# muhanzhang/IGMC

Measured on AMD Instinct MI355X. Metric: enclosing-subgraphs/sec (train step, batch=50) + test RMSE, higher is better.
Workload: dtype f32; 1 GPU; ml_1m, hop 1, max-nodes-per-hop 100, batch 50 per GPU, adj-dropout 0, dynamic-train, ARR 0.001, Adam; parallelism=dp1, global_batch=50, graphs_captured_before_timing=True, steps_per_graph_launch=100, group_steps=50

## Files before the change

### igmc_amd/csrc/capi.hip

```cpp
#include "launch.h"
#include "sortpool.h"
#include "g2_image.h"

#include <algorithm>
#include <climits>
#include <cmath>
#include <cstdio>
#include <cstring>
#include <map>
#include <string>
#include <vector>

static thread_local std::string g_err;
int g_igmc_prof_on = 0;

#define IGMC_FAIL(msg)                                                      \
  do {                                                                      \
    g_err = std::string(__func__) + ": " + (msg);                           \
    return 1;                                                               \
  } while (0)
#define HIPCHECK(expr)                                                      \
  do {                                                                      \
    hipError_t e_ = (expr);                                                 \
    if (e_ != hipSuccess) {                                                 \
// ... 467 lines not shown
      IGMC_FAIL("group extraction needs lean arenas with one control block attached and no side-feature source");
  }
  igmc_launch_extract_set(g->d, s->d_views, b0->d, count, d_link_u, d_link_v, d_link_y, d_link_idx, sel0, B, sample_ratio,
                          seed, b0->ctrl, drop_p, force_undirected, drop_seed, stream);
  HIPCHECK(hipGetLastError());
  for (int i = 0; i < count; ++i) s->arenas[i]->last_B = B;
  return 0;
}

static void ensure_csr(const igmc_batch* b, void* stream) {
  if (b->lean && b->d.relm && b->last_B > 0) igmc_launch_emit(b->d, b->last_B, stream);
}

extern "C" int igmc_batch_assume_size(igmc_batch* b, int B) {
  if (!b) IGMC_FAIL("null batch");
  if (B <= 0 || B > b->d.graph_cap) IGMC_FAIL("batch size out of range");
  b->last_B = B;
  return 0;
}

extern "C" int igmc_batch_set_lean(igmc_batch* b, int lean) {
  if (!b) IGMC_FAIL("null batch");
  b->lean = lean ? 1 : 0;
  return 0;
}

extern "C" int igmc_batch_edge_dropout(igmc_batch* b, float p, int force_undirected, uint64_t seed, uint64_t step,
                                       void* stream) {
  if (!b) IGMC_FAIL("null batch");
  if (b->lean && b->d.relm && b->last_B > 0) {
    igmc_launch_relm_dropout(b->d, b->last_B, p, force_undirected, seed, step, b->ctrl, stream);
  } else {
    igmc_launch_edge_flags(b->d, p, force_undirected, seed, step, b->ctrl, stream);
  }
  HIPCHECK(hipGetLastError());
  return 0;
}

extern "C" int igmc_batch_get_info(const igmc_batch* b, igmc_batch_info* out, void* stream) {
  if (!b || !out) IGMC_FAIL("null argument");
  ensure_csr(b, stream);
  int32_t t[8];
  HIPCHECK(hipStreamSynchronize((hipStream_t)stream));
  HIPCHECK(hipMemcpy(t, b->d.totals, sizeof(t), hipMemcpyDeviceToHost));
  out->num_graphs = t[3];
  out->num_nodes = t[2] ? t[4] : t[0];
  out->num_edges = t[2] ? t[5] : t[1];
  out->overflow = t[2];
  out->node_capacity = b->d.node_cap;
  out->edge_capacity = b->d.edge_cap;
  out->num_labels = b->d.num_labels;
  out->hop = b->d.hop;
  return 0;
}

extern "C" int igmc_batch_set_edge_flags(igmc_batch* b, const uint8_t* h_flags, int64_t n) {
  if (!b || !h_flags) IGMC_FAIL("null argument");
  if (n > b->d.edge_cap) IGMC_FAIL("too many flags");
  ensure_csr(b, nullptr);
  HIPCHECK(hipDeviceSynchronize());
  HIPCHECK(hipMemcpy(b->d.eflag, h_flags, (size_t)n, hipMemcpyHostToDevice));
  igmc_launch_relm_flags(b->d, nullptr);
  HIPCHECK(hipDeviceSynchronize());
  return 0;
}

extern "C" int igmc_batch_clear_edge_flags(igmc_batch* b) {
  if (!b) IGMC_FAIL("null batch");
  igmc_batch_info info;
  if (igmc_batch_get_info(b, &info, nullptr)) return 1;
  if (info.num_edges > 0) {
    HIPCHECK(hipMemset(b->d.eflag, 3, (size_t)info.num_edges));
    igmc_launch_relm_flags(b->d, nullptr);
    HIPCHECK(hipDeviceSynchronize());
  }
  return 0;
}

extern "C" int igmc_batch_download(const igmc_batch* b, int32_t* node_off, int32_t* n_users, uint8_t* node_label,
                                   int32_t* node_gid, int32_t* node_graph, int32_t* row_ptr, int32_t* col,
                                   uint8_t* erel, uint8_t* elab, uint8_t* eflag, float* y, void* stream) {
  igmc_batch_info info;
  if (igmc_batch_get_info(b, &info, stream)) return 1;
  if (info.overflow) IGMC_FAIL("batch arena overflow");
  const int B = info.num_graphs, N = info.num_nodes, E = info.num_edges;
  const BatchDev& d = b->d;
  if (node_off) HIPCHECK(hipMemcpy(node_off, d.node_off, (B + 1) * 4, hipMemcpyDeviceToHost));
  if (n_users) HIPCHECK(hipMemcpy(n_users, d.n_users, B * 4, hipMemcpyDeviceToHost));
  if (node_label && N) HIPCHECK(hipMemcpy(node_label, d.node_label, N, hipMemcpyDeviceToHost));
  if (node_gid && N) HIPCHECK(hipMemcpy(node_gid, d.node_gid, N * 4, hipMemcpyDeviceToHost));
  if (node_graph && N) HIPCHECK(hipMemcpy(node_graph, d.node_graph, N * 4, hipMemcpyDeviceToHost));
  if (row_ptr) HIPCHECK(hipMemcpy(row_ptr, d.row_ptr, (N + 1) * 4, hipMemcpyDeviceToHost));
  if ((col || erel) && E) {
    std::vector<uint32_t> ecr(E);
    HIPCHECK(hipMemcpy(ecr.data(), d.ecr, (size_t)E * 4, hipMemcpyDeviceToHost));
    for (int e = 0; e < E; ++e) {
      if (col) col[e] = (int32_t)(ecr[e] & 0xFFFFFFu);
      if (erel) erel[e] = (uint8_t)(ecr[e] >> 24);
    }
  }
  if (elab && E) {
    std::vector<uint16_t> code(E);
    HIPCHECK(hipMemcpy(code.data(), d.ecode, (size_t)E * 2, hipMemcpyDeviceToHost));
    for (int e = 0; e < E; ++e) elab[e] = (uint8_t)(code[e] % d.num_labels);
  }
  if (eflag && E) HIPCHECK(hipMemcpy(eflag, d.eflag, E, hipMemcpyDeviceToHost));
  if (y) HIPCHECK(hipMemcpy(y, d.y, B * sizeof(float), hipMemcpyDeviceToHost));
  return 0;
}

extern "C" void* igmc_batch_device_ptr(const igmc_batch* b, int which) {
  if (!b) return nullptr;
  const BatchDev& d = b->d;
  switch (which) {
    case IGMC_BUF_NODE_OFF: return d.node_off;
    case IGMC_BUF_N_USERS: return d.n_users;
    case IGMC_BUF_NODE_LABEL: return d.node_label;
    case IGMC_BUF_NODE_GID: return d.node_gid;
    case IGMC_BUF_NODE_GRAPH: return d.node_graph;
    case IGMC_BUF_ROW_PTR: return d.row_ptr;
    case IGMC_BUF_ECR: return d.ecr;
    case IGMC_BUF_ECODE: return d.ecode;
    case IGMC_BUF_EFLAG: return d.eflag;
    case IGMC_BUF_Y: return d.y;
    case IGMC_BUF_TOTALS: return d.totals;
  }
  return nullptr;
}

extern "C" int igmc_batch_set_side_features(igmc_batch* b, const float* d_feat, int n_side) {
  if (!b) IGMC_FAIL("null batch");
  b->side = d_feat;
  b->n_side = n_side;
  b->side_src = nullptr;
  return 0;
}

extern "C" int igmc_batch_bind_side_source(igmc_batch* b, const float* d_side_all, int n_side) {
  if (!b) IGMC_FAIL("null batch");
  if (!d_side_all || n_side <= 0) {
    b->side_src = nullptr;
    b->side = nullptr;
    b->n_side = 0;
    return 0;
  }
  if (b->side_buf_cols < n_side) {
    HIPCHECK(hipSetDevice(b->g->device));
    const int cols = std::max(n_side, 2 * b->side_buf_cols);
    if (b->mem.get(&b->side_buf, (size_t)b->d.graph_cap * cols)) IGMC_FAIL("hipMalloc failed (side features)");
    b->side_buf_cols = cols;
  }
  b->side_src = d_side_all;
  b->side = b->side_buf;
  b->n_side = n_side;
  return 0;
}

extern "C" int igmc_model_create(int device, int num_relations, int num_bases, int num_labels, int n_side,
                                 int max_nodes, int max_edges, int max_graphs, igmc_model** out) {
  if (!out) IGMC_FAIL("null out");
  if (num_bases != 4) IGMC_FAIL("the gfx950 kernels are built for num_bases == 4 (reference Main.py:393)");
  if (num_relations < 1 || num_relations > 255) IGMC_FAIL("num_relations out of range");
  if (num_relations * num_labels + num_labels + 1 > 320) IGMC_FAIL("num_relations * num_labels too large for the layer-0 gradient kernel");
  if (num_labels < 2 || n_side < 0 || max_nodes < 1 || max_graphs < 1) IGMC_FAIL("bad sizes");
  HIPCHECK(hipSetDevice(device));
  igmc_model* m = new igmc_model();
  m->device = device;
  m->last_B = 0;
  m->last_training = 0;
  m->last_flags = 0;
  m->img_valid = 0;
  m->img_hint = 0;
  m->img_params = nullptr;
  ModelDev& d = m->d;
  d.img_current = 0;
  d.adam_m1 = nullptr;
  d.adam_m2 = nullptr;
  d.R = num_relations;
  d.Bs = 4;
  d.L = num_labels;
  d.S = n_side;
  d.D = 256 + n_side;
  int64_t off = 0;
  for (int l = 0; l < 4; ++l) {
    const int fin = l == 0 ? d.L : 32;
    d.off_basis[l] = off; off += (int64_t)4 * fin * 32;
    d.off_root[l] = off;  off += (int64_t)fin * 32;
    d.off_bias[l] = off;  off += 32;
    d.off_att[l] = off;   off += (int64_t)d.R * 4;
  }
  d.off_l1w = off; off += (int64_t)128 * d.D;
  d.off_l1b = off; off += 128;
  d.off_l2w = off; off += 128;
  d.off_l2b = off; off += 1;
  d.n_params = off;
  d.node_cap = max_nodes;
  d.edge_cap = max_edges;
  d.graph_cap = max_graphs;
  Allocs& M = m->mem;
  int fail = 0;
  const size_t N = (size_t)max_nodes, Bc = (size_t)max_graphs;
  for (int l = 0; l < 4; ++l) fail |= M.get(&d.h[l], N * 32) | M.get(&d.dpre[l], N * 32);
  fail |= M.get(&d.agg, N * 128);
  for (int l = 0; l < 3; ++l) fail |= M.get(&d.gagg[l], N * 128) | M.get(&d.Y[l], N * 128);
  fail |= M.get(&d.feat, Bc * d.D) | M.get(&d.a1, Bc * 128) | M.get(&d.lmask, Bc * 128) | M.get(&d.dz, Bc * 128) |
          M.get(&d.gfeat, Bc * d.D) | M.get(&d.err, Bc) | M.get(&d.cnt0, N * d.R * d.L);
  const size_t rows0 = (size_t)d.R * d.L + d.L + 1;
  d.ts_part = nullptr;
  d.ts_raw = nullptr;
  d.ts_stride = (d.R * 32 + 33) * 32;
  d.fin_stash = nullptr;
  d.datt_part = nullptr;
  if (d.R <= G2_NR * G2_NG_MAX)
  {
    fail |= M.get(&d.ts_part, (size_t)4 * IGMC_TS_BLOCKS * d.ts_stride) |
            M.get(&d.ts_raw, (size_t)4 * d.ts_stride + (size_t)4 * d.ts_stride / 32 * 4);
    if (!fail) d.datt_part = d.ts_raw + (size_t)4 * d.ts_stride;
  }
  if (d.R <= 128) fail |= M.get(&d.fin_stash, (size_t)4 * IGMC_STASH_LAYER + 16);
  d.g2_ex = nullptr;
  d.g2_fx = nullptr;
  d.g2_px = nullptr;
  d.g2_px_stride = 0;
  d.g2_w = nullptr;
  d.g2_graphs = 0;
  d.ex_nodes = 256;
  d.g2_ex_stride = (size_t)Bc * 2 * 32 * d.ex_nodes;
  const int wide = d.R <= G2_NR * G2_NG_MAX;
  const int xcd_ok = igmc_g2_xcd_ok();
  if (wide && Bc <= 2048 && xcd_ok) {
    fail |= M.get(&d.g2_ex, 5 * d.g2_ex_stride) | M.get(&d.g2_fx, Bc * 256) | M.get(&d.g2_w, g2_w_words(d.R, d.L));
    d.g2_graphs = (int)Bc;
    if (d.R <= G2_NR && Bc <= 1024) {
      d.g2_px_stride = (size_t)Bc * 2 * 32768;
      fail |= M.get(&d.g2_px, 5 * d.g2_px_stride);
    } else if (d.R <= G2_NR) {
      static bool told = false;
      if (!told) fprintf(stderr, "[igmc] batches of more than 1024 subgraphs: no plane-exchange regions -- the dense-layer / per-layer kernels take the steps, not the subgraph kernel\n");
      told = true;
    }
  } else if (wide) {
    fail |= M.get(&d.g2_w, g2_w_words(d.R, d.L));
  }
  fail |= M.get(&d.gs_bar, 2 * Bc + 1);
  fail |= M.get(&d.gs_ts, 4);
  d.gs_err = d.gs_bar ? d.gs_bar + 2 * Bc : nullptr;
  fail |= M.get(&d.wg_part, (size_t)4 * IGMC_WG_BLOCKS * igmc_wg_stride()) |
          M.get(&d.gatt_part, (size_t)3 * IGMC_GATHER_BLOCKS * d.R * 4) |
          M.get(&d.l0_part, (size_t)IGMC_L0_BLOCKS * rows0 * 32) |
          M.get(&d.graw, (size_t)3 * igmc_wg_stride() + 3 * d.R * 4 + rows0 * 32) | M.get(&d.arr_part, 4);
  d.side = nullptr;
  d.ctrl = nullptr;
  d.dcat[0] = d.dcat[1] = d.dcat[2] = nullptr;
  fail |= M.get(&m->done_ctr, 8);
  if (fail) {
    M.release();
    delete m;
    IGMC_FAIL("hipMalloc failed (model workspace)");
  }
  {
    hipStream_t st1, st2;
    if (hipStreamCreateWithFlags(&st1, hipStreamNonBlocking) != hipSuccess ||
        hipStreamCreateWithFlags(&st2, hipStreamNonBlocking) != hipSuccess) {
      M.release();
      delete m;
      IGMC_FAIL("hipStreamCreate failed");
    }
    m->ax.s1 = st1;
    m->ax.s2 = st2;
    for (int i = 0; i < 8; ++i) {
      hipEvent_t e;
      if (hipEventCreateWithFlags(&e, hipEventDisableTiming) != hipSuccess) IGMC_FAIL("hipEventCreate failed");
      m->ax.ev[i] = e;
    }
  }
  HIPCHECK(hipMemset(m->done_ctr, 0, 8 * sizeof(int)));
  HIPCHECK(hipMemset(m->d.gs_bar, 0, (2 * (size_t)max_graphs + 1) * sizeof(int)));
  {
    const unsigned long long ts0[4] = {~0ull, 0ull, 0ull, 0ull};
    HIPCHECK(hipMemcpy(m->d.gs_ts, ts0, sizeof(ts0), hipMemcpyHostToDevice));
  }
  if (m->d.g2_ex) {
    HIPCHECK(hipMemset(m->d.g2_ex, 0, 5 * m->d.g2_ex_stride * sizeof(unsigned long long)));
    HIPCHECK(hipMemset(m->d.g2_fx, 0, (size_t)max_graphs * 256 * sizeof(unsigned long long)));
    if (m->d.g2_px) HIPCHECK(hipMemset(m->d.g2_px, 0, 5 * m->d.g2_px_stride));
  }
  if (igmc_model_prepare(d)) {
    M.release();
    delete m;
    IGMC_FAIL("hipFuncSetAttribute failed");
  }
  *out = m;
  return 0;
}

extern "C" int igmc_debug_lin_mask(const igmc_model* m, uint8_t* h_out, int64_t n) {
  if (!m || !h_out) IGMC_FAIL("null argument");
  if (n < 0 || n > (int64_t)m->d.graph_cap * 128) IGMC_FAIL("mask size out of range");
  HIPCHECK(hipDeviceSynchronize());
  HIPCHECK(hipMemcpy(h_out, m->d.lmask, (size_t)n, hipMemcpyDeviceToHost));
  return 0;
}

extern "C" void igmc_model_destroy(igmc_model* m) {
  if (!m) return;
  for (int i = 0; i < 8; ++i) hipEventDestroy((hipEvent_t)m->ax.ev[i]);
  hipStreamDestroy((hipStream_t)m->ax.s1);
  hipStreamDestroy((hipStream_t)m->ax.s2);
  m->mem.release();
  delete m;
}

extern "C" int64_t igmc_param_count(const igmc_model* m) { return m ? m->d.n_params : 0; }

extern "C" int64_t igmc_param_offset(const igmc_model* m, int layer, int which, int64_t* count) {
  if (!m) return -1;
  const ModelDev& d = m->d;
  const int fin = (layer == 0) ? d.L : 32;
  int64_t off = -1, n = 0;
  switch (which) {
    case IGMC_P_BASIS: off = d.off_basis[layer & 3]; n = (int64_t)4 * fin * 32; break;
    case IGMC_P_ROOT: off = d.off_root[layer & 3]; n = (int64_t)fin * 32; break;
    case IGMC_P_BIAS: off = d.off_bias[layer & 3]; n = 32; break;
    case IGMC_P_ATT: off = d.off_att[layer & 3]; n = (int64_t)d.R * 4; break;
    case IGMC_P_LIN1_W: off = d.off_l1w; n = (int64_t)128 * d.D; break;
    case IGMC_P_LIN1_B: off = d.off_l1b; n = 128; break;
    case IGMC_P_LIN2_W: off = d.off_l2w; n = 128; break;
    case IGMC_P_LIN2_B: off = d.off_l2b; n = 1; break;
  }
  if (count) *count = n;
  return off;
}

static StepPlan plan_query(const igmc_model* m, const igmc_batch* b, int B) {
  StepPlan sp;
  igmc_step_plan(m->d, b->d, B, IGMC_CALL_STEP, &sp);
  return sp;
}

extern "C" int igmc_model_dense_layers(const igmc_model* m, const igmc_batch* b, int B) {
  return (m && b) ? plan_query(m, b, B).dense_layers : 0;
}

extern "C" int igmc_model_dense_path(const igmc_model* m, const igmc_batch* b, int B) {
  return (m && b) ? plan_query(m, b, B).family == IGMC_FAM_G2 : 0;
}

extern "C" int igmc_model_step_form(const igmc_model* m, const igmc_batch* b, int B) {
  return (m && b) ? plan_query(m, b, B).step_form : 0;
}

extern "C" int igmc_model_step_geometry(const igmc_model* m, const igmc_batch* b, int B, int32_t* out, int n) {
  if (!m || !b || !out || n < 0) IGMC_FAIL("bad arguments");
  if (B < 1 || B > b->d.graph_cap) IGMC_FAIL("batch size outside the arena's capacity");
  const StepPlan sp = plan_query(m, b, B);
  const int g2 = sp.family == IGMC_FAM_G2, dense = sp.family == IGMC_FAM_DLF || sp.family == IGMC_FAM_DL;
  const int32_t v[IGMC_GEOM_N] = {sp.step_form,
                                  sp.family,
                                  g2 ? sp.cs : 0,
                                  g2 ? sp.grid : 0,
                                  sp.nqu,
                                  sp.nqv,
                                  sp.family == IGMC_FAM_ROWS ? 0 : sp.wide ? g2_groups(m->d.R, m->d.L) : 1,
                                  sp.wide && sp.gsplit,
                                  g2 || sp.dlts,
                                  g2 ? sp.lay.kp : 0,
                                  dense && sp.dlb};
  for (int i = 0; i < n && i < IGMC_GEOM_N; ++i) out[i] = v[i];
  return 0;
}

static int check_fit(igmc_model* m, const igmc_batch* b, std::string* why) {
  if (!m || !b) { *why = "null model or batch"; return 1; }
  if (b->last_B <= 0) { *why = "batch is empty (run igmc_extract_batch first)"; return 1; }
  if (b->d.node_cap > m->d.node_cap || b->d.graph_cap > m->d.graph_cap) { *why = "batch capacity exceeds the model workspace"; return 1; }
  if (b->d.num_labels != m->d.L) { *why = "num_labels mismatch (hop)"; return 1; }
  if (b->g->max_rel >= m->d.R) { *why = "graph has more relations than the model"; return 1; }
  if (m->d.S != b->n_side && m->d.S > 0) { *why = "side feature width mismatch"; return 1; }
  return 0;
}

static int check_call(igmc_model* m, const igmc_batch* b, bool buffers, std::string* why) {
  if (check_fit(m, b, why)) return 1;
  if (!buffers) { *why = "null buffer"; return 1; }
  return 0;
}
static StepPlan begin_call(igmc_model* m, const igmc_batch* b, int kind, void* stream) {
  m->d.side = b->side;
  StepPlan sp;
  igmc_step_plan(m->d, b->d, b->last_B, kind, &sp);
  if (b->lean && sp.needs_csr) ensure_csr(b, stream);
  return sp;
}
static void end_call(igmc_model* m, const igmc_batch* b, int training, int use_edge_flags) {
  m->last_B = b->last_B;
  m->last_training = training;
  m->last_flags = use_edge_flags;
}

struct AdamScalars {
  float step_size, inv_sqrt_bc2;
};
static AdamScalars adam_scalars(const int64_t* d_ctrl, int64_t t, float lr, float beta1, float beta2) {
  AdamScalars a = {0.f, 0.f};
  if (!d_ctrl) {
    const double bc1 = 1.0 - std::pow((double)beta1, (double)t);
    const double bc2 = 1.0 - std::pow((double)beta2, (double)t);
    a.step_size = (float)((double)lr / bc1);
    a.inv_sqrt_bc2 = (float)(1.0 / std::sqrt(bc2));
  }
  return a;
}

extern "C" int igmc_model_forward(igmc_model* m, const float* d_params, const igmc_batch* b, int training,
                                  int use_edge_flags, const uint8_t* d_lin_mask, uint64_t seed, uint64_t step,
                                  float multiply_by, float* d_out, void* stream) {
  std::string why;
  if (check_call(m, b, d_params && d_out, &why)) IGMC_FAIL(why);
  const StepPlan sp = begin_call(m, b, training ? IGMC_CALL_CONV : IGMC_CALL_EVAL, stream);
  ImgScope img(m, d_params);
  igmc_launch_forward(m->d, b->d, sp, d_params, b->last_B, training, use_edge_flags, d_lin_mask, seed, step, multiply_by,
                      d_out, stream);
  img.done_unchanged();
  HIPCHECK(hipGetLastError());
  end_call(m, b, training, use_edge_flags);
  return 0;
}

extern "C" int igmc_model_backward(igmc_model* m, const float* d_params, const igmc_batch* b, const float* d_gout,
                                   float multiply_by, float* d_grad, void* stream) {
  std::string why;
  if (check_fit(m, b, &why)) IGMC_FAIL(why);
  if (!m->last_training || m->last_B != b->last_B) IGMC_FAIL("backward needs a preceding training-mode forward on this batch");
  if (!d_params || !d_gout || !d_grad) IGMC_FAIL("null buffer");
  StepPlan sp;
  igmc_step_plan(m->d, b->d, b->last_B, IGMC_CALL_CONV, &sp);
  igmc_launch_backward(m->d, b->d, sp, d_params, b->last_B, m->last_flags, d_gout, 0, 0.f, multiply_by, 2.f, 0.f, d_grad,
                       stream);
  HIPCHECK(hipGetLastError());
  return 0;
}

extern "C" int igmc_model_loss_grad(igmc_model* m, const float* d_params, const igmc_batch* b, int use_edge_flags,
                                    const uint8_t* d_lin_mask, uint64_t seed, uint64_t step, float multiply_by,
                                    float ARR, float grad_scale, float arr_scale, float* d_out, float* d_grad,
                                    float* d_loss, void* stream) {
  std::string why;
  if (check_call(m, b, d_params && d_out && d_grad, &why)) IGMC_FAIL(why);
  const StepPlan sp = begin_call(m, b, IGMC_CALL_STEP, stream);
  ImgScope img(m, d_params);
  igmc_launch_loss_grad(m->d, b->d, sp, (float*)d_params, b->last_B, use_edge_flags, d_lin_mask, seed, step,
                        multiply_by, ARR, grad_scale, arr_scale, d_out, d_grad, d_loss, nullptr, stream);
  img.done_unchanged();
  HIPCHECK(hipGetLastError());
  end_call(m, b, 1, use_edge_flags);
  return 0;
}

extern "C" int igmc_adam_step(float* d_params, const float* d_grad, float* d_exp_avg, float* d_exp_avg_sq, int64_t n,
                              int64_t step, float lr, float beta1, float beta2, float eps, float weight_decay,
                              void* stream) {
  if (!d_params || !d_grad || !d_exp_avg || !d_exp_avg_sq || n <= 0 || step < 1) IGMC_FAIL("bad arguments");
  const AdamScalars as = adam_scalars(nullptr, step, lr, beta1, beta2);
  igmc_launch_adam(d_params, d_grad, d_exp_avg, d_exp_avg_sq, n, as.step_size, as.inv_sqrt_bc2, beta1, beta2, eps, weight_decay,
                   nullptr, 0, stream);
  HIPCHECK(hipGetLastError());
  return 0;
}

extern "C" int igmc_sse_accumulate(const float* d_out, const igmc_batch* b, double* d_acc, void* stream) {
  if (!d_out || !b || !d_acc) IGMC_FAIL("null argument");
  igmc_launch_sse(b->d, d_out, d_acc, nullptr, stream);
  HIPCHECK(hipGetLastError());
  return 0;
}
extern "C" int igmc_sse_accumulate_tick(const float* d_out, const igmc_batch* b, double* d_acc, int64_t* d_ctrl, void* stream) {
  if (!d_out || !b || !d_acc || !d_ctrl) IGMC_FAIL("null argument");
  igmc_launch_sse(b->d, d_out, d_acc, d_ctrl, stream);
  HIPCHECK(hipGetLastError());
  return 0;
}

extern "C" int igmc_scores_store(const float* d_out, const igmc_batch* b, double* d_acc, float* d_scores, float* d_labels,
                                 int64_t n, int64_t first_or_minus1, int64_t* d_ctrl, int32_t* d_err, void* stream) {
  if (!d_out || !b || !d_acc || !d_scores || !d_labels || !d_err) IGMC_FAIL("null argument");
  if (n < 1 || n > (int64_t)INT32_MAX) IGMC_FAIL("n must be in [1, 2^31)");
  if (first_or_minus1 < -1 || first_or_minus1 >= n) IGMC_FAIL("first must be -1 (the arena's stamp) or a position below n");
  igmc_launch_scores_store(b->d, d_out, d_acc, d_ctrl, d_scores, d_labels, n, first_or_minus1, d_err, stream);
  HIPCHECK(hipGetLastError());
  return 0;
}
static int select_grid(int64_t n, int num, int grid) {
  if (n < 1 || n > (int64_t)INT32_MAX || num < 1 || num > IGMC_SELECT_MAX_NUM || grid < 0 || grid > IGMC_SELECT_MAX_GRID) return -1;
  return grid > 0 ? grid : igmc_select_default_grid(n);
}
extern "C" int64_t igmc_select_scratch_bytes(int64_t n, int num, int grid) {
  const int g = select_grid(n, num, grid);
  if (g < 0) {
    g_err = std::string(__func__) + ": n must be in [1, 2^31), num in [1, 64], grid in [0, 1024]";
    return -1;
  }
  return (int64_t)2 * g * num * (int64_t)sizeof(uint64_t);
}
extern "C" int igmc_select_extremes(const float* d_keys, int64_t n, int num, int32_t* d_idx_low, int32_t* d_idx_high,
                                    float* d_key_low, float* d_key_high, int32_t* d_count, void* d_scratch,
                                    int64_t scratch_bytes, int grid, void* stream) {
  if (!d_keys || !d_idx_low || !d_idx_high || !d_scratch) IGMC_FAIL("null argument");
  const int g = select_grid(n, num, grid);
  if (g < 0) IGMC_FAIL("n must be in [1, 2^31), num in [1, 64], grid in [0, 1024]");
  if (scratch_bytes < (int64_t)2 * g * num * (int64_t)sizeof(uint64_t)) IGMC_FAIL("scratch too small (igmc_select_scratch_bytes)");
  if (((uintptr_t)d_scratch & 7) != 0) IGMC_FAIL("scratch must be 8-byte aligned");
  igmc_launch_select(d_keys, n, num, g, d_scratch, d_idx_low, d_idx_high, d_key_low, d_key_high, d_count, stream);
  HIPCHECK(hipGetLastError());
  return 0;
}

extern "C" int igmc_candidates_count(const igmc_graph* g, const int32_t* d_users, int nq, const uint8_t* d_item_ok,
                                     int exclude_seen, int64_t* d_counts, int32_t* d_err, void* stream) {
  if (!g || !d_users || !d_counts || !d_err) IGMC_FAIL("null argument");
  if (nq < 1) IGMC_FAIL("nq must be at least 1");
  igmc_launch_candidates_count(g->d, d_users, nq, d_item_ok, exclude_seen != 0, d_counts, d_err, stream);
  HIPCHECK(hipGetLastError());
  return 0;
}
extern "C" int igmc_candidates_fill(const igmc_graph* g, const int32_t* d_users, int nq, const uint8_t* d_item_ok,
                                    int exclude_seen, const int64_t* d_offsets, int32_t* d_link_u, int32_t* d_link_v,
                                    int64_t capacity, int32_t* d_err, void* stream) {
  if (!g || !d_users || !d_offsets || !d_link_u || !d_link_v || !d_err) IGMC_FAIL("null argument");
  if (nq < 1) IGMC_FAIL("nq must be at least 1");
  if (capacity < 1 || capacity > (int64_t)INT32_MAX) IGMC_FAIL("capacity must be in [1, 2^31)");
  igmc_launch_candidates_fill(g->d, d_users, nq, d_item_ok, exclude_seen != 0, d_offsets, d_link_u, d_link_v, capacity, d_err,
                              stream);
  HIPCHECK(hipGetLastError());
  return 0;
}
static int segsel_split(int ns, int num, int geometry) {
  if (ns < 1 || num < 1 || num > IGMC_SELECT_MAX_NUM || geometry < 0 || geometry > IGMC_SEGSEL_MAX_SPLIT) return -1;
  return geometry > 0 ? geometry : igmc_segsel_default_split(ns);
}
static int64_t segsel_bytes(int ns, int num, int k) {
  return k > 1 ? (int64_t)ns * k * num * (int64_t)sizeof(uint64_t) : (int64_t)sizeof(uint64_t);
}
extern "C" int64_t igmc_select_segments_scratch_bytes(int ns, int num, int geometry) {
  const int k = segsel_split(ns, num, geometry);
  if (k < 0) {
    g_err = std::string(__func__) + ": ns must be at least 1, num in [1, 64], geometry in [0, 64]";
    return -1;
  }
  return segsel_bytes(ns, num, k);
}
extern "C" int igmc_select_segments(const float* d_keys, const int64_t* d_seg_off, int ns, int num, int32_t* d_idx_out,
                                    float* d_key_out, int32_t* d_count, void* d_scratch, int64_t scratch_bytes, int geometry,
                                    void* stream) {
  if (!d_keys || !d_seg_off || !d_idx_out || !d_count || !d_scratch) IGMC_FAIL("null argument");
  const int k = segsel_split(ns, num, geometry);
  if (k < 0) IGMC_FAIL("ns must be at least 1, num in [1, 64], geometry in [0, 64]");
  if (scratch_bytes < segsel_bytes(ns, num, k)) IGMC_FAIL("scratch too small (igmc_select_segments_scratch_bytes)");
  if (((uintptr_t)d_scratch & 7) != 0) IGMC_FAIL("scratch must be 8-byte aligned");
  igmc_launch_select_segments(d_keys, d_seg_off, ns, num, k, d_scratch, d_idx_out, d_key_out, d_count, stream);
  HIPCHECK(hipGetLastError());
  return 0;
}

extern "C" int igmc_ctrl_tick(int64_t* d_ctrl, void* stream) {
  if (!d_ctrl) IGMC_FAIL("null ctrl");
  igmc_launch_tick(d_ctrl, stream);
  HIPCHECK(hipGetLastError());
  return 0;
}
extern "C" int igmc_ctrl_regroup(int64_t* d_ctrl, int M, int64_t first_cur, int64_t first_next, void* stream) {
  if (!d_ctrl || M < 1 || first_cur < 0 || first_next < 0) IGMC_FAIL("bad arguments");
  igmc_launch_regroup(d_ctrl, M, first_cur, first_next, stream);
  HIPCHECK(hipGetLastError());
  return 0;
}
extern "C" int igmc_ctrl_gate(int64_t* d_ctrl, int q, int gk_min, double delay_us, int delay_always, double timeout_us,
                              void* stream) {
  if (!d_ctrl || gk_min < 0 || !(timeout_us >= 0.0) || !(delay_us >= 0.0) || delay_us > 1000.0) IGMC_FAIL("bad arguments");
  igmc_launch_gate(d_ctrl, q & 1, gk_min, (long long)(delay_us * 100.0), delay_always != 0, (long long)(timeout_us * 100.0), stream);
  HIPCHECK(hipGetLastError());
  return 0;
}
extern "C" int igmc_batch_set_ctrl(igmc_batch* b, const int64_t* d_ctrl) {
  if (!b) IGMC_FAIL("null batch");
  b->ctrl = d_ctrl;
  return 0;
}
extern "C" int igmc_model_set_ctrl(igmc_model* m, const int64_t* d_ctrl) {
  if (!m) IGMC_FAIL("null model");
  m->d.ctrl = d_ctrl;
  return 0;
}
extern "C" int igmc_model_reset_exchange(igmc_model* m, void* stream) {
  if (!m) IGMC_FAIL("null model");
  hipStream_t st = (hipStream_t)stream;
  if (m->d.g2_ex) {
    HIPCHECK(hipMemsetAsync(m->d.g2_ex, 0, 5 * m->d.g2_ex_stride * sizeof(unsigned long long), st));
    HIPCHECK(hipMemsetAsync(m->d.g2_fx, 0, (size_t)m->d.g2_graphs * 256 * sizeof(unsigned long long), st));
    if (m->d.g2_px) HIPCHECK(hipMemsetAsync(m->d.g2_px, 0, 5 * m->d.g2_px_stride, st));
  }
  return 0;
}
extern "C" int igmc_model_check(igmc_model* m, void* stream) {
  if (!m) IGMC_FAIL("null model");
  int v = 0;
  if (m->d.gs_err) {
// ... 625 lines not shown
```

### igmc_amd/csrc/g2_subgraph.h

```cpp
#pragma once

struct G2Args {
  const int32_t* n_users;
  const int32_t* n_items;
  int B;
  const uint8_t* s_lab;
  const uint8_t* relm;
  const float* y;
  int cap_u, cap_v, slot, relm_ld, graph_cap;
  int R, L, D, ts_stride;
  float* h[4];
  float* ts_part;
  unsigned char* g2_px;
  unsigned long long* g2_fx;
  size_t g2_px_stride;
  const float* g2_w;
  int* gs_bar;
  int* gs_err;
  float* a1;
  float* dz;
  float* feat;
  float* gfeat;
  float* err;
  uint8_t* lmask;
// ... 4 lines not shown
  const uint8_t* inj_mask;
  uint64_t seed, step;
  float mult, grad_scale;
  float* out;
  unsigned long long* ts;
  int timing, cs, stride, self_seq;
  G2Layout lay2;
};

template <bool FLAGS, bool TRAIN, bool ONCE>
__global__ __launch_bounds__(G2_THREADS) void k_graph_step2(G2Args a) {
  __builtin_amdgcn_s_setprio(3);
  const float* P = a.P;
  IGMC_DYN_SMEM(smem);
  float* S = (float*)smem;
  const G2Layout lay = a.lay2;
  const int kp = lay.kp, nsides = lay.nsides;
  uint32_t* PLN = (uint32_t*)(S + lay.planes);
  uint32_t* OHP = (uint32_t*)(S + lay.ohp);
  unsigned char* slab = (unsigned char*)(S + lay.lab);
  float* XOA = S + lay.xo;
  float* HSS = S + lay.hs;
  float* TILES = S + lay.tile;
  float* HIST = S + lay.hist;
  float* PXA = S + lay.px;
  float2* sW2 = (float2*)(S + lay.wreg);
  float* sT0 = S + lay.t0;
  float* sfeat = S + lay.head;
  float* sgf = sfeat + 256;
  float* sa1 = sgf + 256;
  float* skeep = sa1 + 128;
  float* sdz = skeep + 128;
  float* sred = sdz + 128;
  float* misc = sred + 512;
  const int R = a.R, L = a.L, RL = R * L;
  const int tid = threadIdx.x, lane = tid & 63, wave = tid >> 6;
  const int li = lane & 15, kq = lane >> 4;
  const int B = a.B;
  const int ts = a.ts_stride;
  const int cs = a.cs;
  const int cm = (cs > 1) ? (int)((blockIdx.x >> 3) % cs) : 0;
  const int half = 2 * cs;
  const uint32_t seq = g2_ld_seq(a.gs_bar);
  const uint32_t tag0 = seq * 8u + 1u;
  const uint64_t step = a.ctrl ? (uint64_t)a.ctrl[IGMC_CTRL_STEP] : a.step;
  if (a.ts && tid == 0) g2_clock_open(a.ts);
  auto xtag = [&](int x) { return tag0 + (uint32_t)x; };
  G2_STAMP(0);
  if (a.timing && tid == 0 && blockIdx.x < 1024) {
    g_g2_wg[blockIdx.x][0] = g2_wall_clock();
    g_g2_wg[blockIdx.x][2] = g2_xcc_id();
  }

  const int g_first = (cs > 1) ? (int)(blockIdx.x / (8 * cs)) * 8 + (int)(blockIdx.x & 7) : (int)blockIdx.x;
  const int g_pre = (g_first < a.graph_cap) ? g_first : a.graph_cap - 1;
  const int pre_cu = a.n_users[g_pre], pre_cv = a.n_items[g_pre];
  const int ld = a.relm_ld;
  auto load_label = [&](int g2) {
    const int hi = (tid >> 7) & 1, t7 = tid & 127;
    const int capx = a.cap_u + hi * (a.cap_v - a.cap_u);
    return (int)a.s_lab[(size_t)g2 * a.slot + hi * a.cap_u + ((t7 < capx) ? t7 : 0)];
  };
  int labv_raw = 0;
  if (tid < 256) g2_glds16((const float4*)(a.g2_w + 6 * G2_WIMG) + (tid & ~63), (float4*)sT0 + (tid & ~63), tid & 63);
  const int tslot = (cs > 1) ? g_first + cm * a.stride : (int)blockIdx.x;
  f32x4 acc0 = (f32x4){0.f, 0.f, 0.f, 0.f};
  bool first_graph = true;
  G2_STAMP(1);

  int g = g_first;
  if (g < B) do {
    int tid_g = threadIdx.x;
    G2_OPAQUE(tid_g);
    const int tid = tid_g, lane = tid & 63, wave = tid >> 6;
    const int li = lane & 15, kq = lane >> 4;
    const int bw = wave >> 1, hf = wave & 1;
    const int gw = cm * G2_NB + bw;
    const int side = gw / half, bi = gw - side * half;
    labv_raw = load_label(g);
    uint32_t bw0[G2_KS], bw1[G2_KS];
    {
      const unsigned char* rmg = a.relm + (size_t)g * a.cap_u * ld;
      const uint32_t rrow = (uint32_t)(16 * bi + li);
#pragma unroll
      for (int s = 0; s < G2_KS; ++s) {
        const uint32_t c0 = (uint32_t)(32 * s + 8 * kq);
        if (side == 0) {
          const uint32_t* p4 = (const uint32_t*)(rmg + (rrow * (uint32_t)ld + c0));
          bw0[s] = p4[0];
          bw1[s] = p4[1];
        } else {
          const unsigned char* pc = rmg + (c0 * (uint32_t)ld + rrow);
          bw0[s] = (uint32_t)pc[0] | ((uint32_t)pc[ld] << 8) | ((uint32_t)pc[2 * ld] << 16) | ((uint32_t)pc[3 * ld] << 24);
          bw1[s] = (uint32_t)pc[4 * ld] | ((uint32_t)pc[5 * ld] << 8) | ((uint32_t)pc[6 * ld] << 16) | ((uint32_t)pc[7 * ld] << 24);
        }
      }
    }
    G2_STAMP(48);
    {
      const float4 z4 = make_float4(0.f, 0.f, 0.f, 0.f);
      for (int i = tid; i < 2 * G2_NB * 16 * G2_XP / 4; i += G2_THREADS) ((float4*)XOA)[i] = z4;
      for (int i = tid; i < G2_NB * 16 * G2_XP / 4; i += G2_THREADS) ((float4*)HIST)[i] = z4;
    }
    G2_STAMP(49);
    const int cu = first_graph ? pre_cu : a.n_users[g], cv = first_graph ? pre_cv : a.n_items[g];
    const int n_own = side ? cv : cu, n_opp = side ? cu : cv;
    const int nbs = g * a.slot + (side ? a.cap_u : 0);
    const int nbun = (n_own + 15) >> 4;
    const bool active = bi < nbun;
    const int row0 = 16 * bi;
    const int nks = (n_opp + 31) >> 5;
    const int sx = (nsides == 2) ? side : 0, so = (nsides == 2) ? 1 - side : 0;
    uint32_t* pl = PLN + so * lay.pside;
    uint32_t* ohp = OHP + so * (8 * kp >> 1);
    float* XO0 = XOA + bw * 16 * G2_XP;
    float* XO1 = XOA + (G2_NB + bw) * 16 * G2_XP;
    float* HS = HSS + bw * 16 * G2_XP;
    float* T = TILES + bw * 16 * G2_TP;
    float* HI = HIST + bw * 16 * G2_XP;
    f32x4* PXo = (f32x4*)PXA + (bw * 2 + hf) * 64 + lane;
    const f32x4* PXi = (const f32x4*)PXA + (bw * 2 + (1 - hf)) * 64 + lane;
    const size_t exs = a.g2_px_stride;
    auto px_of = [&](int x, int sd) { return a.g2_px + (size_t)x * exs + ((size_t)g * 2 + sd) * G2_PX_BYTES; };
    unsigned long long* fx = a.g2_fx + (size_t)g * 256;
    const int nbun_opp = (n_opp + 15) >> 4;

    if (tid < 256) slab[tid] = (unsigned char)(((tid & 127) < ((tid >> 7) ? cv : cu)) ? labv_raw : 255);
    G2_STAMP(50);
    __syncthreads();
    G2_STAMP(2);
    {
      for (int i = tid; i < nsides * 8 * (kp >> 1); i += G2_THREADS) {
        const int s2 = i / (8 * (kp >> 1)), rem = i - s2 * (8 * (kp >> 1));
        const int lb = rem / (kp >> 1), q = rem - lb * (kp >> 1);
        const int sd = (nsides == 2) ? s2 : 1 - side;
        const int l0 = (2 * q < 128) ? slab[sd * 128 + 2 * q] : 255, l1 = (2 * q + 1 < 128) ? slab[sd * 128 + 2 * q + 1] : 255;
        OHP[i] = ((l0 == lb) ? 0x3F80u : 0u) | ((l1 == lb) ? 0x3F800000u : 0u);
      }
    }
    __syncthreads();
    G2_STAMP(3);
    uint32_t AM[G2_NR][G2_KS][2];
    uint32_t RB[FLAGS ? G2_KS : 1][2];
    const int kb = side ? IGMC_RELM_KF : IGMC_RELM_KT;
    {
      const int kf = side ? IGMC_RELM_KT : IGMC_RELM_KF;
#pragma unroll
      for (int s = 0; s < G2_KS; ++s) {
        uint32_t w0 = 0u, w1 = 0u;
        if (active && s < nks && row0 + li < n_own) {
          w0 = bw0[s];
          w1 = bw1[s];
          {
            const int keep = n_opp - (32 * s + 8 * kq);
            if (keep < 8) {
              w1 = (keep <= 4) ? 0u : (w1 & (0xFFFFFFFFu >> (8 * (8 - keep))));
              if (keep < 4) w0 = (keep <= 0) ? 0u : (w0 & (0xFFFFFFFFu >> (8 * (4 - keep))));
            }
          }
        }
        if constexpr (FLAGS) {
          RB[s][0] = w0;
          RB[s][1] = w1;
        }
#pragma unroll
        for (int r = 0; r < G2_NR; ++r) {
          AM[r][s][0] = g2_bytemask<FLAGS>(w0, (uint32_t)(r + 1), kf);
          AM[r][s][1] = g2_bytemask<FLAGS>(w1, (uint32_t)(r + 1), kf);
        }
      }
    }
    auto frag_f = [&](int r, int s) {
      uint32_t m0 = AM[r][s][0], m1 = AM[r][s][1];
      G2_OPAQUE(m0);
      G2_OPAQUE(m1);
      return g2_mask_frag(m0, m1);
    };
    auto frag_b = [&](int r, int s) {
      uint32_t m0 = FLAGS ? RB[FLAGS ? s : 0][0] : AM[r][s][0], m1 = FLAGS ? RB[FLAGS ? s : 0][1] : AM[r][s][1];
      G2_OPAQUE(m0);
      G2_OPAQUE(m1);
      if constexpr (FLAGS) return g2_mask_frag(g2_bytemask<true>(m0, (uint32_t)(r + 1), kb), g2_bytemask<true>(m1, (uint32_t)(r + 1), kb));
      else return g2_mask_frag(m0, m1);
    };
    G2_STAMP(4);

    static_assert(G2_WIMG % 256 == 0, "an image is a whole number of 1 KB pieces");
    auto wload = [&](int l, int trans) {
      const float4* src = (const float4*)(a.g2_w + (size_t)((l - 1) * 2 + trans) * G2_WIMG);
#pragma unroll
      for (int j = 0; j < (G2_WIMG / 256 + G2_THREADS / 64 - 1) / (G2_THREADS / 64); ++j) {
        const int c = wave + j * (G2_THREADS / 64);
        if (c < G2_WIMG / 256) g2_glds16(src + c * 64, (float4*)sW2 + c * 64, lane);
      }
    };
    wload(1, 0);
    auto fwd_out = [&](int l, const f32x4& o, float bias, float* XO) {
      const int nt = hf;
      float* hrow = a.h[l] + (size_t)(nbs + row0 + 4 * kq) * 32 + li;
      float* xo = XO + 4 * kq * G2_XP + li;
      float v[4];
#pragma unroll
      for (int rr = 0; rr < 4; ++rr) {
        const float tv = g2_tanh(o[rr] + bias);
        v[rr] = (row0 + 4 * kq + rr < n_own) ? tv : 0.f;
      }
      if (l < 3) {
        g2_publish_planes(px_of(l, side), kp, 16 * nt + li, row0 + 4 * kq, v);
        g2_flag_raise(px_of(l, side), 2 * bi + hf, xtag(l), lane);
      }
#pragma unroll
      for (int rr = 0; rr < 4; ++rr) {
        xo[rr * G2_XP + 16 * nt] = v[rr];
        if (TRAIN && row0 + 4 * kq + rr < n_own) hrow[rr * 32 + 16 * nt] = v[rr];
      }
      if (bi == 0 && kq == 0) g2_pub_f32(fx + side * 128 + l * 32 + 16 * nt + li, v[0], tag0 + G2_FXTAG);
    };
    auto raise = [&](int x) { g2_flag_raise(px_of(x, side), 2 * bi + hf, xtag(x), lane); };
    auto fetch = [&](int x) {
      if (nsides == 1) {
        g2_flags_wait(px_of(x, 1 - side), 2 * nbun_opp, xtag(x), lane, a.gs_err);
        g2_planes_load(PLN, px_of(x, 1 - side), kp, wave, lane, G2_THREADS / 64);
      } else {
        for (int s2 = 0; s2 < 2; ++s2) {
          g2_flags_wait(px_of(x, s2), 2 * (((s2 ? cv : cu) + 15) >> 4), xtag(x), lane, a.gs_err);
          g2_planes_load(PLN + s2 * lay.pside, px_of(x, s2), kp, wave, lane, G2_THREADS / 64);
        }
      }
    };

    if (active) {
      f32x4 hacc[G2_NR];
#pragma unroll
      for (int r = 0; r < G2_NR; ++r) hacc[r] = (f32x4){0.f, 0.f, 0.f, 0.f};
      u32x4 pfh[G2_KS];
#pragma unroll
      for (int s = 0; s < G2_KS; ++s) {
        pfh[s] = *(const u32x4*)(ohp + ((li & 7) * kp >> 1) + 16 * s + 4 * kq);
        if (li >= 8 || s >= nks) pfh[s] = (u32x4){0u, 0u, 0u, 0u};
      }
      G2_SCHED_BARRIER();
#pragma unroll
      for (int s = 0; s < G2_KS; ++s) {
#pragma unroll
        for (int r = 0; r < G2_NR; ++r) {
          hacc[r] = g2_mfma_bf16(pfh[s], frag_f(r, s), hacc[r]);
        }
      }
      G2_STAMP(51);
#pragma unroll
      for (int r = 0; r < G2_NR; ++r)
#pragma unroll
        for (int rr = 0; rr < 4; ++rr)
          if (r < R && 4 * kq + rr < L) HI[li * G2_XP + r * L + 4 * kq + rr] = hacc[r][rr];
      if (kq == 0 && row0 + li < n_own) {
        HI[li * G2_XP + RL + slab[side * 128 + row0 + li]] = 1.f;
        HI[li * G2_XP + RL + L] = 1.f;
      }
      IGMC_WAVE_SYNC();
      f32x4 o = (f32x4){0.f, 0.f, 0.f, 0.f};
#pragma unroll
      for (int j = 0; j < 8; ++j) {
        const float av = HI[li * G2_XP + 4 * j + kq];
        o = __builtin_amdgcn_mfma_f32_16x16x4f32(av, sT0[(4 * j + kq) * 32 + 16 * hf + li], o, 0, 0, 0);
      }
      G2_STAMP(52);
      fwd_out(0, o, 0.f, XO0);
    }
    G2_STAMP(5);

#pragma unroll
    for (int l = 1; l < 4; ++l) {
      float* XOc = (l & 1) ? XO0 : XO1;
      float* XOn = (l & 1) ? XO1 : XO0;
      G2_STAMP(6 + 3 * (l - 1));
      const float bias0 = P[a.off_bias[l] + 16 * hf + li];
      fetch(l - 1);
      if (l > 1) wload(l, 0);
      __syncthreads();
      G2_STAMP(7 + 3 * (l - 1));
      float bias0_ = bias0;
      G2_OPAQUE(bias0_);
      f32x4 o[2];
      if (active) {
        int lane_ = lane;
        G2_OPAQUE(lane_);
        const int li_ = lane_ & 15, kq_ = lane_ >> 4;
        f32x4 acc[G2_NR];
        g2_gather_h(pl, kp, nks, frag_f, li_, kq_, hf, acc);
        if (l == 2) G2_STAMP(40);
        g2_transform_h(acc, XOc, (const uint32_t*)sW2, li_, kq_, hf, o);
        if (l == 2) G2_STAMP(41);
        *PXo = hf ? o[0] : o[1];
      }
      __syncthreads();
      if (l == 2) G2_STAMP(42);
      if (active) {
        const f32x4 po = *PXi;
        f32x4 of;
#pragma unroll
        for (int rr = 0; rr < 4; ++rr) of[rr] = hf ? po[rr] + o[1][rr] : o[0][rr] + po[rr];
        fwd_out(l, of, bias0_, XOn);
      }
      G2_STAMP(36 + (l - 1));
      G2_STAMP(8 + 3 * (l - 1));
    }

    const int ju_h = 16 * wave + ((lane >> 1) & 15);
    float hd_l1b = P[a.off_l1b + ju_h], hd_l2w = P[a.off_l2w + ju_h], hd_l2b = P[a.off_l2b], hd_y = a.y[g];
    float hd_l2wt = TRAIN ? P[a.off_l2w + (tid & 127)] : 0.f;
    if (tid < 256) sfeat[tid] = g2_poll_f32(fx + tid, tag0 + G2_FXTAG, a.gs_err);
    __syncthreads();
    G2_OPAQUE(hd_l1b); G2_OPAQUE(hd_l2w); G2_OPAQUE(hd_l2b); G2_OPAQUE(hd_y); G2_OPAQUE(hd_l2wt);
    G2_STAMP(15);
    float4 w4[16];
    {
      const int ju = 16 * wave + ((lane >> 1) & 15), part = (lane & 1) | (lane >> 5);
      const float4 f4 = *(const float4*)(sfeat + 4 * lane);
      const float* wrow = P + a.off_l1w + (int64_t)(16 * wave) * 256 + 4 * lane;
      float v[16];
      {
#pragma unroll
        for (int q = 0; q < 16; ++q) w4[q] = *(const float4*)(wrow + q * 256);
        G2_SCHED_BARRIER();
#pragma unroll
        for (int q = 0; q < 16; ++q) v[q] = (w4[q].x * f4.x + w4[q].y * f4.y) + (w4[q].z * f4.z + w4[q].w * f4.w);
        G2_SCHED_BARRIER();
      }
#define G2_BFLY(H)                                                                   \
      {                                                                              \
        const bool up = (lane & (2 * (H))) != 0;                                     \
        _Pragma("unroll") for (int i = 0; i < (H); ++i) {                            \
          const float send = up ? v[i] : v[i + (H)], keep = up ? v[i + (H)] : v[i];  \
          v[i] = keep + __shfl_xor(send, 2 * (H));                                   \
        }                                                                            \
      }
      G2_BFLY(8) G2_BFLY(4) G2_BFLY(2) G2_BFLY(1)
#undef G2_BFLY
      float s = v[0] + __shfl_xor(v[0], 1);
      s += __shfl_xor(s, 32);
      G2_STAMP(54);
      if (part == 0) {
        float av = s + hd_l1b;
        av = av > 0.f ? av : 0.f;
        int keep = 1;
        if (TRAIN) {
          keep = a.inj_mask ? (int)a.inj_mask[g * 128 + ju]
                            : (int)(igmc_u01(igmc_unit_hash(a.seed, step, (uint32_t)g, (uint32_t)ju)) >= 0.5f);
          if (cm == 0) {
            a.a1[g * 128 + ju] = av;
            a.lmask[g * 128 + ju] = (uint8_t)keep;
          }
          sa1[ju] = av;
          skeep[ju] = keep ? 1.f : 0.f;
        }
        sred[ju] = (TRAIN ? (keep ? av * 2.f : 0.f) : av) * hd_l2w;
      }
    }
    __syncthreads();
    if (wave == 0) {
      float s = sred[lane] + sred[lane + 64];
      s = igmc_wave_sum_f(s);
      if (lane == 0) {
        const float o = (s + hd_l2b) * a.mult;
        const float e = o - hd_y;
        if (cm == 0) {
          a.out[g] = o;
          a.err[g] = e;
        }
        misc[0] = e;
      }
    }
    if (!TRAIN) {
      first_graph = false;
      __syncthreads();
      continue;
    }
    if (TRAIN) {
      __syncthreads();
      G2_STAMP(16);
      if (tid < 128) {
        const float dp = 2.f * misc[0] * a.grad_scale * a.mult;
        const float dzv = (sa1[tid] > 0.f && skeep[tid] != 0.f) ? dp * hd_l2wt * 2.f : 0.f;
        sdz[tid] = dzv;
        if (cm == 0) a.dz[g * 128 + tid] = dzv;
      }
      if (cm == 0 && tid < 256) a.feat[(size_t)g * a.D + tid] = sfeat[tid];
      __syncthreads();
      {
        float4 s4 = make_float4(0.f, 0.f, 0.f, 0.f);
        const float4* dz4 = (const float4*)(sdz + 16 * wave);
#pragma unroll
        for (int q4 = 0; q4 < 4; ++q4) {
          const float4 d4 = dz4[q4];
          const float dq[4] = {d4.x, d4.y, d4.z, d4.w};
#pragma unroll
          for (int u = 0; u < 4; ++u) {
            const float4 wv = w4[4 * q4 + u];
            s4.x += dq[u] * wv.x; s4.y += dq[u] * wv.y; s4.z += dq[u] * wv.z; s4.w += dq[u] * wv.w;
          }
        }
        *(float4*)(TILES + wave * 256 + 4 * lane) = s4;
      }
      wload(3, 1);
      __syncthreads();
      if (tid < 256) {
        const float v = ((TILES[tid] + TILES[256 + tid]) + (TILES[512 + tid] + TILES[768 + tid])) +
                        ((TILES[1024 + tid] + TILES[1280 + tid]) + (TILES[1536 + tid] + TILES[1792 + tid]));
        sgf[tid] = v;
        if (cm == 0) a.gfeat[(size_t)g * a.D + tid] = v;
      }
      __syncthreads();
      G2_STAMP(17);
      for (int i = tid; i < nsides * G2_NT * 32 * 16; i += G2_THREADS) {
        const int s2 = i / (G2_NT * 32 * 16), r2 = i - s2 * (G2_NT * 32 * 16);
        PLN[s2 * lay.pside + (r2 >> 4) * (kp >> 1) + (r2 & 15)] = 0u;
      }
      for (int i = lane; i < 16 * G2_XP; i += 64) XO0[i] = 0.f;
      __syncthreads();
      if (tid < 32 * nsides) {
        const int s2 = tid >> 5, f = tid & 31;
        const int sd = (nsides == 2) ? s2 : 1 - side;
        const float hv = sfeat[sd * 128 + 96 + f];
        const float d = sgf[sd * 128 + 96 + f] * (1.f - hv * hv);
        uint32_t h, mi, lo;
        g2_split2(d, 0.f, h, mi, lo);
        uint32_t* p2 = PLN + s2 * lay.pside + (f * kp >> 1);
        p2[0] = h & 0xFFFFu;
        p2[32 * kp >> 1] = mi & 0xFFFFu;
        p2[2 * (32 * kp >> 1)] = lo & 0xFFFFu;
      }
      if (active && bi == 0 && lane < 32) {
        const float hv = sfeat[side * 128 + 96 + lane];
        XO0[lane] = sgf[side * 128 + 96 + lane] * (1.f - hv * hv);
      }
      __syncthreads();
      G2_STAMP(18);

#pragma unroll
      for (int l = 3; l >= 1; --l) {
        float* XOc = (l & 1) ? XO0 : XO1;
        float* XOn = (l & 1) ? XO1 : XO0;
        float* wpart = a.ts_part + ((size_t)l * IGMC_TS_BLOCKS + tslot) * ts;
        {
          const int n = tid & 31, part = tid >> 5;
          float sb = 0.f;
          for (int row = part; row < G2_NB * 16; row += G2_THREADS / 32)
            sb += XOA[(((l & 1) ? 0 : G2_NB) + (row >> 4)) * 16 * G2_XP + (row & 15) * G2_XP + n];
          sred[part * 32 + n] = sb;
        }
        __syncthreads();
        if (tid < 32) {
          float s = 0.f;
          for (int p = 0; p < G2_THREADS / 32; ++p) s += sred[p * 32 + tid];
          if (first_graph) wpart[(R * 32 + 32) * 32 + tid] = s;
          else wpart[(R * 32 + 32) * 32 + tid] += s;
        }
        G2_STAMP(19 + 5 * (3 - l));
        float hreg[4];
#pragma unroll
        for (int rr = 0; rr < 4; ++rr) hreg[rr] = 0.f;
        f32x4 o[2];
        if (active) {
          {
            const float* hrow = a.h[l - 1] + (size_t)(nbs + row0 + 4 * kq) * 32 + 16 * hf + li;
#pragma unroll
            for (int rr = 0; rr < 4; ++rr)
              if (row0 + 4 * kq + rr < n_own) hreg[rr] = hrow[rr * 32];
          }
          int lane_ = lane;
          G2_OPAQUE(lane_);
          const int li_ = lane_ & 15, kq_ = lane_ >> 4;
          f32x4 acc[G2_NR];
          if (l == 2) G2_STAMP(43);
          g2_gather_h(pl, kp, (l == 3) ? 1 : nks, frag_b, li_, kq_, hf, acc);
          if (l == 2) G2_STAMP(44);
#pragma unroll
          for (int r = 0; r < G2_NR; ++r)
            *(float4*)(T + li * G2_TP + r * 32 + 16 * hf + 4 * kq) = make_float4(acc[r][0], acc[r][1], acc[r][2], acc[r][3]);
#pragma unroll
          for (int rr = 0; rr < 4; ++rr) HS[(4 * kq + rr) * G2_XP + 16 * hf + li] = hreg[rr];
          if (l == 2) G2_STAMP(45);
          g2_transform_h(acc, XOc, (const uint32_t*)sW2, li_, kq_, hf, o);
          if (l == 2) G2_STAMP(46);
          *PXo = hf ? o[0] : o[1];
#pragma unroll
          for (int rr = 0; rr < 4; ++rr) G2_OPAQUE(hreg[rr]);
        } else if (hf == 0) {
          for (int i = lane; i < 16 * G2_TP; i += 64) T[i] = 0.f;
          for (int i = lane; i < 16 * G2_XP; i += 64) HS[i] = 0.f;
        }
        __syncthreads();
        if (l == 2) G2_STAMP(47);
        if (active) {
          const f32x4 po = *PXi;
          const int f = 16 * hf + li;
          float v[4];
#pragma unroll
          for (int rr = 0; rr < 4; ++rr) {
            const int row = 4 * kq + rr;
            float d = hf ? po[rr] + o[1][rr] : o[0][rr] + po[rr];
            if (bi == 0 && row == 0) d += sgf[side * 128 + (l - 1) * 32 + f];
            const float x = hreg[rr];
            v[rr] = (row0 + row < n_own) ? d * (1.f - x * x) : 0.f;
          }
          if (l > 1) {
            g2_publish_planes(px_of(6 - l, side), kp, f, row0 + 4 * kq, v);
            raise(6 - l);
          }
#pragma unroll
          for (int rr = 0; rr < 4; ++rr) XOn[(4 * kq + rr) * G2_XP + f] = v[rr];
        }
        G2_STAMP(20 + 5 * (3 - l));
        G2_STAMP(21 + 5 * (3 - l));
        if (l > 1) wload(l - 1, 1);
        {
          f32x4 w3[3];
#pragma unroll
          for (int i3 = 0; i3 < 3; ++i3) w3[i3] = (f32x4){0.f, 0.f, 0.f, 0.f};
          const int m2w = wave >> 2, wo = wave & 3;
#pragma unroll 1
          for (int wb = 0; wb < G2_NB; ++wb) {
            const float* Tb = TILES + wb * 16 * G2_TP;
            const float* Hb = HSS + wb * 16 * G2_XP;
            const float* Db = XOA + (((l & 1) ? 0 : G2_NB) + wb) * 16 * G2_XP;
            float av[4], bw3[4][3];
#pragma unroll
            for (int s4 = 0; s4 < 4; ++s4) {
              av[s4] = Hb[(4 * s4 + kq) * G2_XP + m2w * 16 + li];
              const float* tb = Tb + (4 * s4 + kq) * G2_TP + li;
              const float* db = Db + (4 * s4 + kq) * G2_XP + li;
#pragma unroll
              for (int i3 = 0; i3 < 3; ++i3) {
                const int nt = 3 * wo + i3;
                bw3[s4][i3] = (nt < 2 * G2_NR) ? tb[nt * 16] : db[(nt - 2 * G2_NR) * 16];
              }
            }
            G2_SCHED_BARRIER();
#pragma unroll
            for (int s4 = 0; s4 < 4; ++s4)
#pragma unroll
              for (int i3 = 0; i3 < 3; ++i3)
                w3[i3] = __builtin_amdgcn_mfma_f32_16x16x4f32(av[s4], bw3[s4][i3], w3[i3], 0, 0, 0);
          }
#pragma unroll
          for (int i3 = 0; i3 < 3; ++i3) {
            const int m2 = m2w, nt = 3 * wo + i3;
            const int r = nt >> 1;
            if (r >= R && r < G2_NR) continue;
            float* pp = wpart + (kq * 4) * 32 + li + (r < R ? r : R) * 1024 + m2 * 512 + (nt & 1) * 16;
            if (first_graph) {
#pragma unroll
              for (int rr = 0; rr < 4; ++rr) pp[rr * 32] = w3[i3][rr];
            } else {
#pragma unroll
              for (int rr = 0; rr < 4; ++rr) pp[rr * 32] += w3[i3][rr];
            }
          }
        }
        G2_STAMP(22 + 5 * (3 - l));
        if (l > 1) fetch(6 - l);
        __syncthreads();
        G2_STAMP(23 + 5 * (3 - l));
      }

      if (wave < 4) {
        const int m2 = wave >> 1, wn = wave & 1;
        for (int wb = 0; wb < G2_NB; ++wb) {
          const float* Hb = HIST + wb * 16 * G2_XP;
          const float* Db = XOA + (G2_NB + wb) * 16 * G2_XP;
#pragma unroll
          for (int s4 = 0; s4 < 4; ++s4)
            acc0 = __builtin_amdgcn_mfma_f32_16x16x4f32(Hb[(4 * s4 + kq) * G2_XP + m2 * 16 + li],
                                                        Db[(4 * s4 + kq) * G2_XP + wn * 16 + li], acc0, 0, 0, 0);
        }
      }
      first_graph = false;
      __syncthreads();
      G2_STAMP(34);
    }
  } while (!ONCE && (g += (int)gridDim.x) < B);

  if (TRAIN && wave < 4) {
    float* part0 = a.ts_part + (size_t)tslot * ts;
    const int m2 = wave >> 1, wn = wave & 1;
#pragma unroll
    for (int rr = 0; rr < 4; ++rr) {
      const int c = m2 * 16 + kq * 4 + rr;
      if (c < RL + L + 1) part0[c * 32 + wn * 16 + li] = acc0[rr];
    }
  }
  if (tid == 0 && a.self_seq) {
    const unsigned long long t1 = a.ts ? g2_wall_clock() : 0ull;
    if (g2_last_workgroup_advances(a.gs_bar) && a.ts) g2_clock_close(a.ts, t1);
  }
  G2_STAMP(35);
  if (a.timing && tid == 0 && blockIdx.x < 1024) g_g2_wg[blockIdx.x][1] = g2_wall_clock();
}

extern "C" int igmc_debug_g2_wg_clocks(unsigned long long* out, int n_wg) {
#ifndef IGMC_HIPEMU
  if (n_wg > 1024) n_wg = 1024;
  if (hipDeviceSynchronize() != hipSuccess) return 1;
  if (hipMemcpyFromSymbol(out, HIP_SYMBOL(g_g2_wg), (size_t)n_wg * 3 * sizeof(unsigned long long)) != hipSuccess) return 1;
#else
  for (int i = 0; i < 3 * n_wg; ++i) out[i] = 0;
#endif
  return 0;
}

extern "C" int igmc_debug_g2_clocks(unsigned long long* out, int n) {
#ifndef IGMC_HIPEMU
  if (n > 128) n = 128;
  if (hipDeviceSynchronize() != hipSuccess) return 1;
  if (hipMemcpyFromSymbol(out, HIP_SYMBOL(g_g2_clk), (size_t)n * sizeof(unsigned long long)) != hipSuccess) return 1;
#else
  for (int i = 0; i < n; ++i) out[i] = 0;
#endif
  return 0;
}
```

Measured before the change: 793,900 subgraphs/s.

## Move backward scratch zeroing into forward tail and fuse bias-grad column sums

Zeroing of the plane and XO0 scratch buffers moves from the start of the backward pass into the end of the forward layer-3 iteration, which removes one block-wide barrier. The per-layer bias-gradient column reduction, previously a separate shared-memory sweep plus barrier, now comes from wave-level shuffles of values already in registers, written into double-buffered sred slots and summed by 32 threads. A debug export of the head arrays is also added. The risk is correctness, since it depends on sred indexing per block-wave (bw), on G2_NB being 4, and on ordering between the early zeroing and later reads.

New measurement: 805,000 subgraphs/s (median of 6 runs). +1.4%, better.

```diff
diff --git a/igmc_amd/csrc/capi.hip b/igmc_amd/csrc/capi.hip
--- a/igmc_amd/csrc/capi.hip
+++ b/igmc_amd/csrc/capi.hip
@@ -793,6 +793,16 @@
   return 0;
 }
 
+extern "C" int igmc_debug_head_array(const igmc_model* m, int which, float* h_out, int64_t n) {
+  if (!m || !h_out) IGMC_FAIL("null argument");
+  if (which < 0 || which > 3) IGMC_FAIL("no such array");
+  const float* src = which == 0 ? m->d.a1 : which == 1 ? m->d.dz : which == 2 ? m->d.feat : m->d.gfeat;
+  if (n < 0 || n > (int64_t)m->d.graph_cap * (which < 2 ? 128 : m->d.D)) IGMC_FAIL("size out of range");
+  HIPCHECK(hipDeviceSynchronize());
+  HIPCHECK(hipMemcpy(h_out, src, (size_t)n * sizeof(float), hipMemcpyDeviceToHost));
+  return 0;
+}
+
 extern "C" void igmc_model_destroy(igmc_model* m) {
   if (!m) return;
   for (int i = 0; i < 8; ++i) hipEventDestroy((hipEvent_t)m->ax.ev[i]);
diff --git a/igmc_amd/csrc/g2_subgraph.h b/igmc_amd/csrc/g2_subgraph.h
--- a/igmc_amd/csrc/g2_subgraph.h
+++ b/igmc_amd/csrc/g2_subgraph.h
@@ -330,6 +330,14 @@
         for (int rr = 0; rr < 4; ++rr) of[rr] = hf ? po[rr] + o[1][rr] : o[0][rr] + po[rr];
         fwd_out(l, of, bias0_, XOn);
       }
+      if (TRAIN && l == 3) {
+        G2_STAMP(39);
+        for (int i = tid; i < nsides * G2_NT * 32 * 16; i += G2_THREADS) {
+          const int s2 = i / (G2_NT * 32 * 16), r2 = i - s2 * (G2_NT * 32 * 16);
+          PLN[s2 * lay.pside + (r2 >> 4) * (kp >> 1) + (r2 & 15)] = 0u;
+        }
+        for (int i = lane + 64 * hf; i < 16 * G2_XP; i += 128) XO0[i] = 0.f;
+      }
       G2_STAMP(36 + (l - 1));
       G2_STAMP(8 + 3 * (l - 1));
     }
@@ -440,12 +448,6 @@
       }
       __syncthreads();
       G2_STAMP(17);
-      for (int i = tid; i < nsides * G2_NT * 32 * 16; i += G2_THREADS) {
-        const int s2 = i / (G2_NT * 32 * 16), r2 = i - s2 * (G2_NT * 32 * 16);
-        PLN[s2 * lay.pside + (r2 >> 4) * (kp >> 1) + (r2 & 15)] = 0u;
-      }
-      for (int i = lane; i < 16 * G2_XP; i += 64) XO0[i] = 0.f;
-      __syncthreads();
       if (tid < 32 * nsides) {
         const int s2 = tid >> 5, f = tid & 31;
         const int sd = (nsides == 2) ? s2 : 1 - side;
@@ -458,9 +460,11 @@
         p2[32 * kp >> 1] = mi & 0xFFFFu;
         p2[2 * (32 * kp >> 1)] = lo & 0xFFFFu;
       }
-      if (active && bi == 0 && lane < 32) {
+      if (hf == 0 && lane < 32) {
         const float hv = sfeat[side * 128 + 96 + lane];
-        XO0[lane] = sgf[side * 128 + 96 + lane] * (1.f - hv * hv);
+        const float d = (active && bi == 0) ? sgf[side * 128 + 96 + lane] * (1.f - hv * hv) : 0.f;
+        if (active && bi == 0) XO0[lane] = d;
+        sred[(1 * G2_NB + bw) * 32 + lane] = d;
       }
       __syncthreads();
       G2_STAMP(18);
@@ -470,20 +474,6 @@
         float* XOc = (l & 1) ? XO0 : XO1;
         float* XOn = (l & 1) ? XO1 : XO0;
         float* wpart = a.ts_part + ((size_t)l * IGMC_TS_BLOCKS + tslot) * ts;
-        {
-          const int n = tid & 31, part = tid >> 5;
-          float sb = 0.f;
-          for (int row = part; row < G2_NB * 16; row += G2_THREADS / 32)
-            sb += XOA[(((l & 1) ? 0 : G2_NB) + (row >> 4)) * 16 * G2_XP + (row & 15) * G2_XP + n];
-          sred[part * 32 + n] = sb;
-        }
-        __syncthreads();
-        if (tid < 32) {
-          float s = 0.f;
-          for (int p = 0; p < G2_THREADS / 32; ++p) s += sred[p * 32 + tid];
-          if (first_graph) wpart[(R * 32 + 32) * 32 + tid] = s;
-          else wpart[(R * 32 + 32) * 32 + tid] += s;
-        }
         G2_STAMP(19 + 5 * (3 - l));
         float hreg[4];
 #pragma unroll
@@ -538,6 +528,20 @@
           }
 #pragma unroll
           for (int rr = 0; rr < 4; ++rr) XOn[(4 * kq + rr) * G2_XP + f] = v[rr];
+          if (l > 1) {
+            float cb = (v[0] + v[1]) + (v[2] + v[3]);
+            cb += __shfl_xor(cb, 16);
+            cb += __shfl_xor(cb, 32);
+            if (kq == 0) sred[(((l - 1) & 1) * G2_NB + bw) * 32 + f] = cb;
+          }
+        } else if (l > 1 && lane < 16) {
+          sred[(((l - 1) & 1) * G2_NB + bw) * 32 + 16 * hf + lane] = 0.f;
+        }
+        if (tid < 32) {
+          const float* sb = sred + (l & 1) * G2_NB * 32 + tid;
+          const float sv = (sb[0] + sb[32]) + (sb[64] + sb[96]);
+          if (first_graph) wpart[(R * 32 + 32) * 32 + tid] = sv;
+          else wpart[(R * 32 + 32) * 32 + tid] += sv;
         }
         G2_STAMP(20 + 5 * (3 - l));
         G2_STAMP(21 + 5 * (3 - l));
```
